# Bernat-C/MRI-Diffusion-SuperResolution

Hardware: AMD Instinct MI355X
Metric: MRI slices/sec (50-step DDIM, 256^2, bs=32) (higher is better)
Workload: dtype bf16; 1 GPU; configs[1]: 256x256 1-ch synthetic MRI slices -> 4x32x32 latents, SD-1.5-size UNet (859.5M params, random init) + rank-4 LoRA, 50-step DDIM, bs=32 per GPU; ddim_steps=50, parallelism=slice-sharded x1 (no collective), lora=explicit adapters, down-projection + rank-r update inside the projection GEMMs, tile_table=profiles/r03_tune_cache.tsv, hipgraph=True

## Files before the change

include/mrisr_debug.h:

```cpp
#ifndef MRISR_DEBUG_H
#define MRISR_DEBUG_H
#ifdef __cplusplus
extern "C" {
#endif

void mrisr_debug_force_split(int splitk);
void mrisr_debug_force_tile(int tile);
void mrisr_debug_prefer_tile(int tile);
void mrisr_debug_gemm_flags(int flags);
void mrisr_debug_set_tile_eff(int tile, double eff);
void mrisr_debug_set_tuned(const char* key, int tile, int splitk);
void mrisr_debug_gn_fused(int on);

int mrisr_autotune_stats(int* shapes, double* ms);
void mrisr_autotune_release(void);

int mrisr_bench_gemm(int M, int N, int K, int conv, int B, int H, int W, int stride, int ups, int c1, int tile, int splitk,
                     int iters, float* ms_out);

void mrisr_debug_sk_inkernel(int on);

void mrisr_debug_subpix(int min_rows);

void mrisr_debug_temb_table(int on);

void mrisr_debug_mlp_proj(int on);

void mrisr_debug_gn_slabs(int on);

void mrisr_debug_xattn_tail(int on);
void mrisr_debug_xattn_tail_stamps(void* dev_buf);

int mrisr_bench_mlp(int M, int hidden, int iters, float* ms_out);

#ifdef __cplusplus
}
#endif
#endif
```

mri-diffusion-superresolution_amd/csrc/common.h:

```cpp
#pragma once
#include <hip/hip_runtime.h>
#include <stdint.h>
#include <string>

namespace mrisr {

typedef __bf16 bf16;
typedef __attribute__((ext_vector_type(8))) __bf16 bf16x8;
typedef __attribute__((ext_vector_type(4))) __bf16 bf16x4;
typedef __attribute__((ext_vector_type(4))) float f32x4;
typedef __attribute__((ext_vector_type(16))) float f32x16;

enum DType : int { DT_F32 = 0, DT_BF16 = 1, DT_F16 = 2, DT_I64 = 3 };

template <typename T> struct TypeTag;
template <> struct TypeTag<float> { static constexpr int id = DT_F32; };
template <> struct TypeTag<bf16> { static constexpr int id = DT_BF16; };

__device__ __forceinline__ float to_f32(float x) { return x; }
__device__ __forceinline__ float to_f32(bf16 x) { return (float)x; }
template <typename T> __device__ __forceinline__ T from_f32(float x);
template <> __device__ __forceinline__ float from_f32<float>(float x) { return x; }
template <> __device__ __forceinline__ bf16 from_f32<bf16>(float x) { return (bf16)x; }

// ... 53 lines not shown
struct GemmArgs {
    const void* a0 = nullptr;
    const void* a1 = nullptr;
    int c0 = 0, c1 = 0;
    int lda0 = 0, lda1 = 0;
    int conv = 0;
    int B = 0, Hin = 0, Win = 0, Hout = 0, Wout = 0, stride = 1, ups = 0;
    int pad = 1;
    int zstuff = 0;
    const void* w = nullptr;
    int M = 0, N = 0, K = 0;
    int kw = 3, subpix = 0;
    int batch = 1;
    long long a_bs = 0, w_bs = 0;
    int heads = 1;
    long long o_bs = 0, o_hs = 0;
    int splitk = 1;
    float* partial = nullptr;
    unsigned* sk_counters = nullptr;
    int defer_reduce = 0;
    int pretouch = 0;
    float alpha = 1.0f;
    const float* bias = nullptr;
    const float* rowvec = nullptr;
    int rowvec_div = 1, rowvec_ld = 0;
    int act = ACT_NONE;
    const void* resid = nullptr;
    int ldr = 0;
    int out_mode = OUT_ROWS;
    void* out = nullptr;
    int ldo = 0;
    void* sec_ptr[3] = {nullptr, nullptr, nullptr};
    int sec_tr[3] = {0, 0, 0};
    int secC = 0, hd = 0, dpad = 0, ntok = 0, npad = 0, nheads = 0;
    double alg_flops = 0.0, alg_bytes = 0.0;
    int tile = 0;
    int stage_out = 1;
    const float* lora_z = nullptr;
    const float* lora_b = nullptr;
    int lora_r = 0, lora_zld = 0, lora_secN = 1;
    const void* lora_a = nullptr;
    int lora_R = 0;
    float* lora_zout = nullptr;
    const float* ln_gamma = nullptr;
    const float* ln_beta = nullptr;
    float ln_eps = 1e-5f;
    const void* w8 = nullptr;
    const float* w_scale = nullptr;
    const void* lora_a8 = nullptr;
    const float* lora_a_scale = nullptr;
    int no_rp = 0;
    int group_m = 1;
    int dbg = 0;
};

template <typename T> int launch_gemm(const GemmArgs& g, hipStream_t st);
template <typename T> int launch_splitk_reduce(const GemmArgs& g, hipStream_t st);
const void* zero_page();
int init_zero_page();
int gemm_prepare();
struct MlpArgs {
    const void* x = nullptr; int ldx = 0, M = 0;
    const float* ln_gamma = nullptr; const float* ln_beta = nullptr; float ln_eps = 1e-5f;
    const void* w1 = nullptr; const float* b1 = nullptr;
    const void* w2p = nullptr; const float* b2 = nullptr;
    const void* resid = nullptr; int ldr = 0;
    void* out = nullptr; int ldo = 0;
    int C = 0, H = 0, N2 = 0;
    const void* wp = nullptr; const float* bp = nullptr;
    const void* xres = nullptr; int ldxr = 0;
    void* out2 = nullptr; int ldo2 = 0;
};
bool mlp_fused_ok(int C, int H, int N2);
bool mlp_proj_enabled();
int launch_pack_mlp_w2(const void* w2_bf16, void* dst, int N2, int H, hipStream_t st);
int launch_mlp_fused(const MlpArgs& m, hipStream_t st);
struct XTailArgs {
    const void* ao = nullptr; int ldao = 0;
    void* t = nullptr; int ldt = 0;
    int M = 0, ntok = 0;
    const void* w1 = nullptr; const float* b1 = nullptr; const void* a1 = nullptr; const float* lb1 = nullptr;
    const float* ln_g = nullptr; const float* ln_b = nullptr; float ln_eps = 1e-5f;
    const void* wq = nullptr; const float* bq = nullptr; const void* aq = nullptr; const float* lbq = nullptr;
    const void* kvp = nullptr; int nk = 0; float scale = 1.f;
    const void* w2 = nullptr; const float* b2 = nullptr; const void* a2 = nullptr; const float* lb2 = nullptr;
    int lora_r = 0;
};
int xattn_tail_prepare();
bool xattn_tail_enabled();
bool xattn_tail_ok(int C, int heads, int M, int ntok, int nk);
size_t xattn_tail_kv_bytes(int B);
int launch_pack_xattn_kv(const void* kc, const void* vtc, void* dst, int B, int ctx_pad, int dpad, int nk, hipStream_t st);
int launch_xattn_tail(const XTailArgs& x, hipStream_t st);
int gemm_rp_tile(const GemmArgs& g);
int gemm_choose(GemmArgs& g, bool is_bf16);

struct GroupNormArgs {
    const void* x0 = nullptr;
    const void* x1 = nullptr;
    int c0 = 0, c1 = 0;
    int B = 0, HW = 0, groups = 32;
    float eps = 1e-5f;
    const float* gamma = nullptr;
    const float* beta = nullptr;
    int silu = 0;
    void* y = nullptr;
// ... 182 lines not shown
```

mri-diffusion-superresolution_amd/csrc/gemm.hip:

```cpp
#include "common.h"
#include "prof.h"

#include <cstdio>
#include <cstdlib>
#include <cstring>
#include <map>
#include <mutex>
#include <unordered_map>

namespace mrisr {

static void* g_zero_page = nullptr;
static constexpr size_t kZeroPageBytes = 128 * 1024;
const void* zero_page() { return g_zero_page; }
int init_zero_page() {
    if (g_zero_page) return 0;
    MRISR_CHECK_HIP(hipMalloc(&g_zero_page, kZeroPageBytes));
    MRISR_CHECK_HIP(hipMemset(g_zero_page, 0, kZeroPageBytes));
    return 0;
}

typedef const __attribute__((address_space(1))) void* gptr_t;
typedef __attribute__((address_space(3))) void* lptr_t;

// ... 115 lines not shown
    if (g.out_mode == OUT_NONE) {
        if (v[0] == 1.2345e30f) store4<T>(reinterpret_cast<T*>(g.out), v);
    } else if (g.out_mode == OUT_ROWS) {
        if (lds_dst) store4<T>(lds_dst, v);
        else store4<T>(reinterpret_cast<T*>(g.out) + zoff + (size_t)m * g.ldo + n0, v);
    } else if (g.out_mode == OUT_F32) {
        store4<float>(reinterpret_cast<float*>(g.out) + zoff + (size_t)m * g.ldo + n0, v);
    } else {
        if (lds_dst) {
            store4<T>(lds_dst, v);
            return;
        }
        if (sizeof(T) == 2 && lds_t) {
            unsigned w0, w1;
            const int drow = exchange_tokens4(v, w0, w1);
            *reinterpret_cast<uint2*>(lds_t + (nl + drow) * tpitch + (ml & ~3)) = make_uint2(w0, w1);
            return;
        }
        const int s = n0 / g.secC;
        const int c = n0 - s * g.secC;
        const int h = c / g.hd;
        const int dd = c - h * g.hd;
        const int b = m / g.ntok;
        const int tok = m - b * g.ntok;
        T* base = reinterpret_cast<T*>(s == 0 ? g.sec_ptr[0] : (s == 1 ? g.sec_ptr[1] : g.sec_ptr[2]));
        const int tr = (s == 0 ? g.sec_tr[0] : (s == 1 ? g.sec_tr[1] : g.sec_tr[2]));
        const size_t bh = (size_t)b * g.nheads + h;
        if (!tr) {
            store4<T>(base + (bh * g.npad + tok) * g.dpad + dd, v);
        } else if (sizeof(T) == 2 && mfma_lanes && (g.ntok & 3) == 0 && (g.M & 3) == 0) {
            unsigned w0, w1;
            const int drow = exchange_tokens4(v, w0, w1);
            T* o = base + (bh * g.dpad + dd + drow) * g.npad + (tok & ~3);
            *reinterpret_cast<uint2*>(o) = make_uint2(w0, w1);
        } else {
            T* o = base + (bh * g.dpad + dd) * g.npad + tok;
#pragma unroll
            for (int r = 0; r < 4; ++r) o[(size_t)r * g.npad] = from_f32<T>(v[r]);
        }
    }
}

template <int NFR>
__device__ __forceinline__ void preload_cols(const GemmArgs& g, int nbase, float (&pb)[NFR][4]) {
    const bool fold = g.rowvec && g.rowvec_div >= g.M;
#pragma unroll
    for (int i = 0; i < NFR; ++i) {
        const int n = min(nbase + i * 16, g.N - 4);
        float b[4] = {0.f, 0.f, 0.f, 0.f}, t[4] = {0.f, 0.f, 0.f, 0.f};
        if (g.bias) load4<float>(g.bias + n, b);
        if (fold) load4<float>(g.rowvec + n, t);
#pragma unroll
        for (int r = 0; r < 4; ++r) pb[i][r] = b[r] + t[r];
    }
}

template <typename T> struct Frag;
template <> struct Frag<bf16> { typedef bf16x8 type; };
template <> struct Frag<float> { typedef f32x4 type; };

__device__ __forceinline__ void mma(f32x4& acc, const bf16x8& w, const bf16x8& a) {
    acc = __builtin_amdgcn_mfma_f32_16x16x32_bf16(w, a, acc, 0, 0, 0);
}
__device__ __forceinline__ void mma(f32x4& acc, const f32x4& w, const f32x4& a) {
#pragma unroll
    for (int j = 0; j < 4; ++j) acc = __builtin_amdgcn_mfma_f32_16x16x4f32(w[j], a[j], acc, 0, 0, 0);
}

__device__ __forceinline__ void lds_poison(char* smem_base, int nthreads) {
    const unsigned bytes = ((const __attribute__((address_space(4))) unsigned*)__builtin_amdgcn_dispatch_ptr())[7];
    for (unsigned o = threadIdx.x * 16u; o + 16u <= bytes; o += (unsigned)nthreads * 16u)
        *reinterpret_cast<uint4*>(smem_base + o) = make_uint4(~0u, ~0u, ~0u, ~0u);
    __syncthreads();
}
static int gemm_flags_now();

template <typename T, int BM, int BN, int WGM, int WGN>
__global__ __launch_bounds__(256) void gemm_kernel(const GemmArgs g, const char* __restrict__ zero) {
    constexpr int EB = sizeof(T);
    constexpr int CH = 16 / EB;
    constexpr int BK = 8 * CH;
    constexpr int A_IT = BM / 32, W_IT = BN / 32;
    constexpr int WTM = BM / WGM, WTN = BN / WGN;
    constexpr int MF = WTM / 16, NF = WTN / 16;
    constexpr int STAGE = (BM + BN) * 128;
    static_assert(WGM * WGN == 4, "4 waves");
    extern __shared__ __attribute__((aligned(16))) char smem[];

    const int tid = threadIdx.x;
    const int lane = tid & 63;
    const int wave = __builtin_amdgcn_readfirstlane(tid >> 6);
    const int z = blockIdx.z;
    const int split = blockIdx.y;
    if (g.dbg & 2048) lds_poison(smem, (int)blockDim.x);

    const int ntn = (g.N + BN - 1) / BN;
    const int ntm = (g.M + BM - 1) / BM;
    const int nblk = ntn * ntm;
    int logical;
    {
        const int bid = blockIdx.x;
        const int xcd = bid & 7, q = nblk >> 3, r = nblk & 7;
        logical = (xcd < r ? xcd * (q + 1) : r * (q + 1) + (xcd - r) * q) + (bid >> 3);
    }
    int tn, tm;
    {
// ... 237 lines not shown
template <int BM, int BN>
__device__ __forceinline__ void copy_out_heads(const GemmArgs& g, const bf16* otile, int m0, int n0, bool tr) {
    __syncthreads();
    const int s = n0 / g.secC;
    bf16* base = reinterpret_cast<bf16*>(s == 0 ? g.sec_ptr[0] : (s == 1 ? g.sec_ptr[1] : g.sec_ptr[2]));
    if (!tr) {
        constexpr int CPR = BN / 8, P = BN + 8;
        for (int idx = threadIdx.x; idx < BM * CPR; idx += 256) {
            const int row = idx / CPR, ch = idx - row * CPR;
            const int m = m0 + row, n = n0 + ch * 8;
            if (m >= g.M || n >= g.N) continue;
            const int c = n - s * g.secC, h = c / g.hd, dd = c - h * g.hd;
            const int b = m / g.ntok, tok = m - b * g.ntok;
            *reinterpret_cast<bf16x8*>(base + (((size_t)b * g.nheads + h) * g.npad + tok) * g.dpad + dd) =
                *reinterpret_cast<const bf16x8*>(otile + row * P + ch * 8);
        }
    } else {
        constexpr int TPC = BM / 8, P = BM + 8;
        for (int idx = threadIdx.x; idx < BN * TPC; idx += 256) {
            const int col = idx / TPC, tc = idx - col * TPC;
            const int n = n0 + col, m = m0 + tc * 8;
            if (m >= g.M || n >= g.N) continue;
            const int c = n - s * g.secC, h = c / g.hd, dd = c - h * g.hd;
            const int b = m / g.ntok, tok = m - b * g.ntok;
            *reinterpret_cast<bf16x8*>(base + (((size_t)b * g.nheads + h) * g.dpad + dd) * g.npad + tok) =
                *reinterpret_cast<const bf16x8*>(otile + col * P + tc * 8);
        }
    }
}

typedef __attribute__((address_space(3))) void* lds_ptr_t;
__device__ __forceinline__ __amdgpu_buffer_rsrc_t make_rsrc(const void* p, unsigned bytes) {
    return __builtin_amdgcn_make_buffer_rsrc(const_cast<void*>(p), 0, bytes, 0x00020000);
}
__device__ __forceinline__ void bl16(__amdgpu_buffer_rsrc_t r, char* lds_wave_base, unsigned voff, unsigned soff) {
    __builtin_amdgcn_raw_ptr_buffer_load_lds(r, (lds_ptr_t)lds_wave_base, 16, voff, soff, 0, 0);
}
#define BL_OOB 0x80000000u


__device__ __forceinline__ void pretouch_weights(const __amdgpu_buffer_rsrc_t& rw, long long w_bytes, char* scratch, int wave, int lane, int cap) {
    const int n_wg = (int)(gridDim.x * gridDim.y);
    const int wg = (int)(blockIdx.x + blockIdx.y * gridDim.x);
    const long long pieces = (w_bytes + 1023) >> 10;
    const int per_wg = (int)((pieces + n_wg - 1) / n_wg);
    const int per_wave = min((per_wg + 3) >> 2, cap);
    const long long first = (long long)wg * per_wg + (long long)wave * per_wave;
    for (int i = 0; i < per_wave; ++i) {
        const long long pc = first + i;
        const unsigned off = pc < pieces ? (unsigned)(pc << 10) + (unsigned)lane * 16u : BL_OOB;
        bl16(rw, scratch + ((wave * 2 + (i & 1)) << 10), off, 0u);
    }
}

template <int NF, int MF>
__device__ __forceinline__ bool splitk_last_arriver(const GemmArgs& g, f32x4 (&acc)[NF][MF], unsigned tile_idx, const float* slab0, int m_base, int n_base,
                                                    int fr, int fg, char* ticket_lds) {
    __builtin_amdgcn_fence(__ATOMIC_RELEASE, "agent");
    __syncthreads();
    if (threadIdx.x == 0)
        *reinterpret_cast<volatile unsigned*>(ticket_lds) = __hip_atomic_fetch_add(g.sk_counters + tile_idx, 1u, __ATOMIC_ACQ_REL, __HIP_MEMORY_SCOPE_AGENT);
    __syncthreads();
    const unsigned ticket = *reinterpret_cast<volatile unsigned*>(ticket_lds);
    if (ticket != (unsigned)g.splitk - 1) return false;
    __syncthreads();
    if (threadIdx.x == 0) __hip_atomic_store(g.sk_counters + tile_idx, 0u, __ATOMIC_RELAXED, __HIP_MEMORY_SCOPE_AGENT);
    __builtin_amdgcn_fence(__ATOMIC_ACQUIRE, "agent");
    const size_t slab = (size_t)g.M * g.N;
#pragma unroll
    for (int i = 0; i < NF; ++i)
#pragma unroll
        for (int j = 0; j < MF; ++j) acc[i][j] = f32x4{0.f, 0.f, 0.f, 0.f};
    for (int s = 0; s < g.splitk; ++s) {
        const float* p = slab0 + (size_t)s * slab;
#pragma unroll
        for (int i = 0; i < NF; ++i)
#pragma unroll
            for (int j = 0; j < MF; ++j) {
                const int m = m_base + j * 16 + fr;
                const int n = n_base + i * 16 + fg * 4;
                if (m < g.M && n < g.N) {
                    const f32x4 t = __builtin_nontemporal_load(reinterpret_cast<const f32x4*>(p + (size_t)m * g.N + n));
                    acc[i][j] += t;
                }
            }
    }
    return true;
}

template <int BM, int BN, int WGM, int WGN, int NSTAGE, bool LORA>
__global__ __launch_bounds__(256, 2) void gemm_bl_kernel(const GemmArgs g) {
    static_assert(NSTAGE >= 2 && NSTAGE <= 4, "2 (drain per tile), 3 or 4 (counted ring)");
    typedef bf16 T;
    constexpr int BK = 64;
    constexpr int A_IT = BM / 32, W_IT = BN / 32;
    constexpr int WTM = BM / WGM, WTN = BN / WGN;
    constexpr int MF = WTM / 16, NF = WTN / 16;
    constexpr int STAGE = (BM + BN) * 128 + (LORA ? 16 * 128 : 0);
    static_assert(WGM * WGN == 4, "4 waves");
    extern __shared__ __attribute__((aligned(16))) char smem[];

    const int tid = threadIdx.x;
    const int lane = tid & 63;
    const int wave = __builtin_amdgcn_readfirstlane(tid >> 6);
    const int z = blockIdx.z;
    const int split = blockIdx.y;
    if (g.dbg & 2048) lds_poison(smem, (int)blockDim.x);

    const int ntn = (g.N + BN - 1) / BN;
    const int ntm = (g.M + BM - 1) / BM;
    const int nblk = ntn * ntm;
    int logical;
    {
        const int bid = blockIdx.x;
        const int xcd = bid & 7, q = nblk >> 3, r = nblk & 7;
        logical = (xcd < r ? xcd * (q + 1) : r * (q + 1) + (xcd - r) * q) + (bid >> 3);
    }
    int tn, tm;
    {
        const int GM = g.group_m > 1 ? g.group_m : 1;
        const int per_group = GM * ntn;
        const int grp = logical / per_group;
        const int first_m = grp * GM;
        const int gsz = min(GM, ntm - first_m);
        const int within = logical - grp * per_group;
        tm = first_m + within % gsz;
        tn = within / gsz;
    }
    const int m0 = tm * BM, n0 = tn * BN;

    const T* a0p = reinterpret_cast<const T*>(g.a0) + (size_t)z * g.a_bs;
    const T* a1p = reinterpret_cast<const T*>(g.a1);
    const T* wp = reinterpret_cast<const T*>(g.w) + (size_t)z * g.w_bs;
    const long long a_rows = g.conv ? (long long)g.B * g.Hin * g.Win : (long long)g.M;
    const __amdgpu_buffer_rsrc_t rw = make_rsrc(wp, (unsigned)min((long long)g.N * g.K * 2, 0x7FFFFFFFll));
    const __amdgpu_buffer_rsrc_t ra0 = make_rsrc(a0p, (unsigned)min(a_rows * g.lda0 * 2, 0x7FFFFFFFll));
    const __amdgpu_buffer_rsrc_t ra1 = make_rsrc(a1p ? (const void*)a1p : (const void*)a0p,
                                                 a1p ? (unsigned)min(a_rows * g.lda1 * 2, 0x7FFFFFFFll) : 0u);

    const int lrow = tid >> 3, pch = tid & 7;
    unsigned wvo[W_IT];
#pragma unroll
    for (int it = 0; it < W_IT; ++it) {
        const int row = it * 32 + lrow;
        const int n = n0 + row;
        const int c = pch ^ (row & 7);
        wvo[it] = n < g.N ? (unsigned)(((size_t)n * g.K + c * 8) * 2) : BL_OOB;
    }
    unsigned avo[A_IT], avo1[A_IT];
    int ab[A_IT], ay[A_IT], ax[A_IT];
#pragma unroll
    for (int it = 0; it < A_IT; ++it) {
        const int row = it * 32 + lrow;
        const int m = m0 + row;
        const int c = pch ^ (row & 7);
        const bool ok = m < g.M;
        avo[it] = avo1[it] = BL_OOB;
        ab[it] = -1;
        ay[it] = ax[it] = 0;
// ... 66 lines not shown
                for (int it = 0; it < A_IT; ++it) {
                    const int row = it * 32 + lrow;
                    const int c = pch ^ (row & 7);
                    const int iy = ay[it] + ky, ix = ax[it] + kx;
                    const bool ok = ab[it] >= 0 && iy >= 0 && iy < Hc && ix >= 0 && ix < Wc && (!g.zstuff || ((iy | ix) & 1) == 0);
                    const unsigned pix = (unsigned)((ab[it] + (iy >> g.ups)) * g.Win + (ix >> g.ups));
                    avo[it] = ok ? (pix * (unsigned)ld + (unsigned)c * 8u) * 2u : BL_OOB;
                }
            }
            const unsigned chb = (unsigned)(second ? cc - g.c0 : cc) * 2;
            if (!second) {
#pragma unroll
                for (int it = 0; it < A_IT; ++it) bl16(ra0, sb + (it * 256 + wave * 64) * 16, avo[it], chb);
            } else {
#pragma unroll
                for (int it = 0; it < A_IT; ++it) bl16(ra1, sb + (it * 256 + wave * 64) * 16, avo[it], chb);
            }
            cc += BK;
            if (cc >= Ct) { cc = 0; ++tap; }
        }
    };
    auto stage = [&](int kt, int buf) { stage_w(kt, buf); stage_a(kt, buf); };
    (void)acb;

    f32x4 acc[NF][MF];
#pragma unroll
    for (int i = 0; i < NF; ++i)
#pragma unroll
        for (int j = 0; j < MF; ++j) acc[i][j] = f32x4{0.f, 0.f, 0.f, 0.f};

    const int wm0 = (wave / WGN) * WTM, wn0 = (wave % WGN) * WTN;
    const int fr = lane & 15, fg = lane >> 4;
    const bool zwave = LORA && (wave % WGN) == 0;
    const bool lora_mma = LORA && g.lora_r == 4 && g.alpha == 1.0f && !(g.dbg & 8);
    bf16x8 lbf[NF];
    if (LORA) {
#pragma unroll
        for (int i = 0; i < NF; ++i) {
            lbf[i] = bf16x8{0, 0, 0, 0, 0, 0, 0, 0};
            const int n = n0 + wn0 + i * 16 + fr;
            if (lora_mma && n < g.N) {
                const int sec = n / g.lora_secN;
                if ((sec >> 1) == fg) {
                    const f32x4 l = *reinterpret_cast<const f32x4*>(g.lora_b + (size_t)n * 4);
                    if (sec & 1) { lbf[i][4] = (bf16)l[0]; lbf[i][5] = (bf16)l[1]; lbf[i][6] = (bf16)l[2]; lbf[i][7] = (bf16)l[3]; }
                    else { lbf[i][0] = (bf16)l[0]; lbf[i][1] = (bf16)l[1]; lbf[i][2] = (bf16)l[2]; lbf[i][3] = (bf16)l[3]; }
                }
            }
        }
    }
    f32x4 zacc[MF];
#pragma unroll
    for (int j = 0; j < MF; ++j) zacc[j] = f32x4{0.f, 0.f, 0.f, 0.f};

    auto compute = [&](int buf, auto&& mid) {
        const char* sa = smem + buf * STAGE;
        const char* sw = sa + BM * 128;
#pragma unroll
        for (int kk = 0; kk < 2; ++kk) {
            if (kk == 1) mid();
            const int phys = ((kk * 4 + fg) ^ (fr & 7)) * 16;
            bf16x8 wf[NF], af[MF];
#pragma unroll
            for (int i = 0; i < NF; ++i) wf[i] = *reinterpret_cast<const bf16x8*>(sw + (wn0 + i * 16 + fr) * 128 + phys);
#pragma unroll
            for (int j = 0; j < MF; ++j) af[j] = *reinterpret_cast<const bf16x8*>(sa + (wm0 + j * 16 + fr) * 128 + phys);
#pragma unroll
            for (int i = 0; i < NF; ++i)
#pragma unroll
                for (int j = 0; j < MF; ++j) acc[i][j] = __builtin_amdgcn_mfma_f32_16x16x32_bf16(wf[i], af[j], acc[i][j], 0, 0, 0);
            if (LORA && zwave) {
                const bf16x8 lf = *reinterpret_cast<const bf16x8*>(sw + (BN + fr) * 128 + phys);
#pragma unroll
                for (int j = 0; j < MF; ++j) zacc[j] = __builtin_amdgcn_mfma_f32_16x16x32_bf16(lf, af[j], zacc[j], 0, 0, 0);
            }
        }
    };

    if constexpr (NSTAGE == 2) {
        if (kt_beg < kt_end) {
            if (g.pretouch) pretouch_weights(rw, (long long)g.N * g.K * 2, smem + STAGE, wave, lane, g.pretouch);
            stage(kt_beg, 0);
            asm volatile("s_waitcnt vmcnt(0)" ::: "memory");
            __syncthreads();
            int cur = 0;
            const bool halves = (g.dbg & 16384) != 0;
            for (int kt = kt_beg; kt < kt_end; ++kt) {
                const bool more = kt + 1 < kt_end;
                if (more) { if (halves) stage_w(kt + 1, cur ^ 1); else stage(kt + 1, cur ^ 1); }
                compute(cur, [&]() {
                    if (halves) {
                        __builtin_amdgcn_sched_barrier(0);
                        if (more) stage_a(kt + 1, cur ^ 1);
                        __builtin_amdgcn_sched_barrier(0);
                    }
                });
                asm volatile("s_waitcnt vmcnt(0)" ::: "memory");
                __syncthreads();
                cur ^= 1;
            }
        }
    } else {
        constexpr int PER = A_IT + W_IT + (LORA ? 1 : 0);
        static_assert(PER * (NSTAGE - 2) <= 63, "vmcnt range");
#pragma unroll
        for (int s = 0; s < NSTAGE - 1; ++s)
            if (kt_beg + s < kt_end) stage(kt_beg + s, s);
        int slot = 0;
        for (int kt = kt_beg; kt < kt_end; ++kt) {
            const int younger = min(NSTAGE - 2, kt_end - 1 - kt);
            if (younger >= 2) asm volatile("s_waitcnt vmcnt(%0)" ::"n"(PER * 2) : "memory");
            else if (younger == 1) asm volatile("s_waitcnt vmcnt(%0)" ::"n"(PER) : "memory");
            else asm volatile("s_waitcnt vmcnt(0)" ::: "memory");
            asm volatile("s_waitcnt lgkmcnt(0)" ::: "memory");
            __builtin_amdgcn_s_barrier();
            if (kt + NSTAGE - 1 < kt_end) stage(kt + NSTAGE - 1, (slot + NSTAGE - 1) % NSTAGE);
            compute(slot, []() {});
            slot = slot + 1 == NSTAGE ? 0 : slot + 1;
        }
        __syncthreads();
    }

    float* zlds = reinterpret_cast<float*>(smem);
    if (LORA) {
        if (zwave) {
#pragma unroll
            for (int j = 0; j < MF; ++j) {
                const int ml = wm0 + j * 16 + fr;
                *reinterpret_cast<f32x4*>(zlds + ml * 16 + fg * 4) = zacc[j];
                if (g.lora_zout && tn == 0 && m0 + ml < g.M && fg * 4 < g.lora_R)
                    *reinterpret_cast<f32x4*>(g.lora_zout + (size_t)(m0 + ml) * g.lora_R + fg * 4) = zacc[j];
            }
        }
        __syncthreads();
    }
    if (LORA && lora_mma) {
        bf16x8 zf[MF];
#pragma unroll
        for (int j = 0; j < MF; ++j) {
            zf[j] = bf16x8{0, 0, 0, 0, 0, 0, 0, 0};
            if (fg < 2) {
                const float* zp = zlds + (wm0 + j * 16 + fr) * 16 + fg * 8;
                const f32x4 a = *reinterpret_cast<const f32x4*>(zp), b = *reinterpret_cast<const f32x4*>(zp + 4);
                zf[j] = bf16x8{(bf16)a[0], (bf16)a[1], (bf16)a[2], (bf16)a[3], (bf16)b[0], (bf16)b[1], (bf16)b[2], (bf16)b[3]};
            }
        }
#pragma unroll
        for (int i = 0; i < NF; ++i)
#pragma unroll
            for (int j = 0; j < MF; ++j) acc[i][j] = __builtin_amdgcn_mfma_f32_16x16x32_bf16(lbf[i], zf[j], acc[i][j], 0, 0, 0);
    }
    if (g.splitk > 1) {
        float* part = g.partial + ((size_t)z * g.splitk + split) * (size_t)g.M * g.N;
#pragma unroll
        for (int i = 0; i < NF; ++i)
#pragma unroll
            for (int j = 0; j < MF; ++j) {
                const int m = m0 + wm0 + j * 16 + fr;
                const int n = n0 + wn0 + i * 16 + fg * 4;
                if (m < g.M && n < g.N) {
                    float v[4] = {acc[i][j][0], acc[i][j][1], acc[i][j][2], acc[i][j][3]};
                    store4<float>(part + (size_t)m * g.N + n, v);
                }
            }
        if constexpr (NF * MF > 20) return;
        else {
            if (!g.sk_counters) return;
            if (!splitk_last_arriver<NF, MF>(g, acc, (unsigned)(z * gridDim.x + blockIdx.x), g.partial + (size_t)z * g.splitk * (size_t)g.M * g.N,
                                             m0 + wm0, n0 + wn0, fr, fg, smem))
                return;
        }
    }
    float pb[NF][4];
    preload_cols<NF>(g, n0 + wn0 + fg * 4, pb);
    if (g.act == ACT_GEGLU) {
        if constexpr (NF % 2 == 0) {
#pragma unroll
            for (int i = 0; i < NF; i += 2)
#pragma unroll
                for (int j = 0; j < MF; ++j) {
                    const int m = m0 + wm0 + j * 16 + fr;
                    const int n = n0 + wn0 + i * 16 + fg * 4;
                    if (m < g.M && n < g.N) {
                        float v[4] = {acc[i][j][0], acc[i][j][1], acc[i][j][2], acc[i][j][3]};
                        float vg[4] = {acc[i + 1][j][0], acc[i + 1][j][1], acc[i + 1][j][2], acc[i + 1][j][3]};
                        epilogue4<T>(g, z, m, n, v, vg, nullptr, nullptr, false, true, nullptr, 0, 0, 0, pb[i], pb[i + 1]);
                    }
                }
        }
        return;
    }
    constexpr int OPITCH = BN + 8;
    T* otile = reinterpret_cast<T*>(smem + (LORA ? BM * 16 * 4 : 0));
    const bool staged = g.out_mode == OUT_ROWS && (g.ldo & 7) == 0 && g.heads == 1 && g.stage_out;
    const bool resid_later = staged && g.resid != nullptr && (g.ldr & 7) == 0 && g.stage_out < 3;
    bool hstaged = false, htr = false;
    if (g.out_mode == OUT_HEADS && g.stage_out && !(g.dbg & 16)) {
        const int sec = n0 / g.secC;
        hstaged = (min(n0 + BN, g.N) - 1) / g.secC == sec && ((g.N | g.M | g.hd | g.secC | g.dpad | g.npad | g.ntok) & 7) == 0 && g.heads == 1 &&
                  g.batch == 1;
        htr = (sec == 0 ? g.sec_tr[0] : (sec == 1 ? g.sec_tr[1] : g.sec_tr[2])) != 0;
    }
#pragma unroll
    for (int i = 0; i < NF; ++i)
#pragma unroll
        for (int j = 0; j < MF; ++j) {
            const int m = m0 + wm0 + j * 16 + fr;
            const int n = n0 + wn0 + i * 16 + fg * 4;
            if (m < g.M && n < g.N) {
                float v[4] = {acc[i][j][0], acc[i][j][1], acc[i][j][2], acc[i][j][3]};
                epilogue4<T>(g, z, m, n, v, nullptr, LORA && !lora_mma ? zlds + (m - m0) * 16 : nullptr,
                             staged || (hstaged && !htr) ? otile + (m - m0) * OPITCH + (n - n0) : nullptr, resid_later, true,
                             hstaged && htr ? otile : nullptr, m - m0, n - n0, BM + 8, pb[i]);
            }
        }
    if (staged) copy_out_tile<BM, BN>(g, otile, OPITCH, m0, n0, z, resid_later);
    else if (hstaged) copy_out_heads<BM, BN>(g, otile, m0, n0, htr);
}

template <int BM, int BN, int WGM, int WGN>
__global__ __launch_bounds__(256, 2) void gemm_halo_kernel(const GemmArgs g) {
    typedef bf16 T;
    constexpr int BK = 64;
    constexpr int W_IT = BN / 32;
    constexpr int WTM = BM / WGM, WTN = BN / WGN;
    constexpr int MF = WTM / 16, NF = WTN / 16;
    constexpr int WSTAGE = BN * 128;
    constexpr int PIT_MAX = (BM >= 256 ? 13 : (BM >= 128 ? 9 : 6));
    static_assert(WGM * WGN == 4, "4 waves");
    extern __shared__ __attribute__((aligned(16))) char smem[];

    const int tid = threadIdx.x;
    const int lane = tid & 63;
    const int wave = __builtin_amdgcn_readfirstlane(tid >> 6);
    const int split = blockIdx.y;
    if (g.dbg & 2048) lds_poison(smem, (int)blockDim.x);
    const int Wd = g.Win, Hd = g.Hin;
    const int TH = BM / Wd, PW = Wd + 2;
    const int npix = (TH + 2) * PW;
    const int pit = (npix * 8 + 255) / 256;
    char* patch = smem;
    char* wbase = smem + pit * 4096;

    const int ntn = (g.N + BN - 1) / BN;
    const int ntm = g.M / BM;
    const int nblk = ntn * ntm;
    int logical;
    {
        const int bid = blockIdx.x;
        const int xcd = bid & 7, q = nblk >> 3, r = nblk & 7;
        logical = (xcd < r ? xcd * (q + 1) : r * (q + 1) + (xcd - r) * q) + (bid >> 3);
    }
    int tn, tm;
    {
        const int GM = g.group_m > 1 ? g.group_m : 1;
        const int per_group = GM * ntn;
        const int grp = logical / per_group;
        const int first_m = grp * GM;
        const int gsz = min(GM, ntm - first_m);
        const int within = logical - grp * per_group;
        tm = first_m + within % gsz;
        tn = within / gsz;
    }
    const int m0 = tm * BM, n0 = tn * BN;
    const int img = m0 / (Hd * Wd);
    const int y0 = (m0 - img * Hd * Wd) / Wd;

    const T* a0p = reinterpret_cast<const T*>(g.a0);
    const T* a1p = reinterpret_cast<const T*>(g.a1);
    const T* wp = reinterpret_cast<const T*>(g.w);
// ... 1453 lines not shown
}

static int auto_group_m(int ntm, int ntn, int BM, int BN) {
    (void)ntn; (void)BM; (void)BN;
    static const int env = [] { const char* e = getenv("MRISR_GROUP_M"); return e ? atoi(e) : 8; }();
    return std::max(1, std::min(env, ntm));
}

template <typename T, int BM, int BN, int WGM, int WGN>
static int prepare_cfg() {
    constexpr int smem = 2 * (BM + BN) * 128;
    static bool attr_set = false;
    if (!attr_set) {
        auto kern = gemm_kernel<T, BM, BN, WGM, WGN>;
        MRISR_CHECK_HIP(hipFuncSetAttribute((const void*)kern, hipFuncAttributeMaxDynamicSharedMemorySize, smem));
        attr_set = true;
    }
    return 0;
}
template <typename T>
static int prepare_all() {
    if (prepare_cfg<T, 128, 128, 2, 2>()) return 1;
    if (prepare_cfg<T, 256, 64, 4, 1>()) return 1;
    if (prepare_cfg<T, 128, 64, 2, 2>()) return 1;
    if (prepare_cfg<T, 64, 64, 2, 2>()) return 1;
    return 0;
}
template <typename T, int BM, int BN, int WGM, int WGN>
static int launch_cfg(const GemmArgs& g, hipStream_t st) {
    constexpr int smem = 2 * (BM + BN) * 128;
    auto kern = gemm_kernel<T, BM, BN, WGM, WGN>;
    if (prepare_cfg<T, BM, BN, WGM, WGN>()) return 1;
    const int ntn = (g.N + BN - 1) / BN, ntm = (g.M + BM - 1) / BM;
    const_cast<GemmArgs&>(g).group_m = auto_group_m(ntm, ntn, BM, BN);
    dim3 grid(ntn * ntm, g.splitk, g.batch);
    static const std::string pname = std::string("gemm_") + (sizeof(T) == 2 ? "bf16_" : "f32_") + std::to_string(BM) + "x" + std::to_string(BN);
    double fl = g.alg_flops, by = g.alg_bytes;
    if (prof_enabled()) {
        if (fl == 0.0) fl = 2.0 * g.M * (double)g.N * g.K * g.batch;
        if (by == 0.0) {
            const double a_el = g.conv ? (double)g.B * g.Hin * g.Win * (g.c0 + g.c1) : (double)g.M * g.K;
            by = sizeof(T) * g.batch * (a_el + (double)g.N * g.K + (double)g.M * g.N);
        }
    }
    ProfScope ps(pname.c_str(), fl, by, st);
    hipLaunchKernelGGL(kern, grid, dim3(256), smem, st, g, (const char*)zero_page());
    MRISR_CHECK_HIP(hipGetLastError());
    return 0;
}

static int g_force_tile = 0;
extern "C" void mrisr_debug_force_tile(int t) { g_force_tile = t; }

template <int BM, int BN, int WGM, int WGN, int NSTAGE>
static int prepare_bl() {
    constexpr int smem = NSTAGE * (BM + BN) * 128;
    constexpr int smem_l = NSTAGE * ((BM + BN) * 128 + 16 * 128);
    static bool done = false;
    if (!done) {
        MRISR_CHECK_HIP(hipFuncSetAttribute((const void*)gemm_bl_kernel<BM, BN, WGM, WGN, NSTAGE, false>, hipFuncAttributeMaxDynamicSharedMemorySize, smem));
        MRISR_CHECK_HIP(hipFuncSetAttribute((const void*)gemm_bl_kernel<BM, BN, WGM, WGN, NSTAGE, true>, hipFuncAttributeMaxDynamicSharedMemorySize, smem_l));
        done = true;
    }
    return 0;
}
template <int BM, int BN, int WGM, int WGN, int NSTAGE>
static int launch_bl(const GemmArgs& g, hipStream_t st) {
    constexpr int smem = NSTAGE * (BM + BN) * 128;
    constexpr int smem_l = NSTAGE * ((BM + BN) * 128 + 16 * 128);
    if (prepare_bl<BM, BN, WGM, WGN, NSTAGE>()) return 1;
    if (NSTAGE > 2)
        MRISR_REQUIRE(!g.conv && !g.c1 && !g.a1 && g.batch == 1 && (g.splitk == 1 || (g.K / 64) / g.splitk >= NSTAGE) && g.M % BM == 0 && g.N % BN == 0,
                      "counted-ring GEMM: plain single-source GEMM that tiles exactly; split: at least NSTAGE K tiles per split");
    const int ntn = (g.N + BN - 1) / BN, ntm = (g.M + BM - 1) / BM;
    const_cast<GemmArgs&>(g).group_m = auto_group_m(ntm, ntn, BM, BN);
    dim3 grid(ntn * ntm, g.splitk, g.batch);
    static const std::string base_name = std::string("gemm_bf16_bl") + std::to_string(BM) + "x" + std::to_string(BN) + (NSTAGE > 2 ? "d" + std::to_string(NSTAGE) : std::string());
    std::string pname = base_name;
    if (prof_enabled() && prof_shapes()) {
        char buf[160];
        snprintf(buf, sizeof(buf), "%s %s M=%d N=%d K=%d s=%d b=%d", base_name.c_str(), g.conv ? (g.ups ? "convup" : (g.stride == 2 ? "convs2" : "conv")) : "lin",
                 g.M, g.N, g.K, g.splitk, g.batch);
        pname = buf;
    }
    double fl = g.alg_flops, by = g.alg_bytes;
    if (prof_enabled()) {
        if (fl == 0.0) fl = 2.0 * g.M * (double)g.N * g.K * g.batch;
        if (by == 0.0) {
            const double a_el = g.conv ? (double)g.B * g.Hin * g.Win * (g.c0 + g.c1) : (double)g.M * g.K;
            by = 2.0 * g.batch * (a_el + (double)g.N * g.K + (double)g.M * g.N);
        }
    }
    ProfScope ps(prof_intern(pname), fl, by, st);
    if (g.lora_a) {
        MRISR_REQUIRE(g.splitk == 1 && !g.conv && g.c1 == 0 && g.lora_R >= 1 && g.lora_R <= 16 && g.lora_b && g.act != ACT_GEGLU,
                      "in-kernel LoRA down-projection: plain un-split GEMM, R <= 16");
        hipLaunchKernelGGL((gemm_bl_kernel<BM, BN, WGM, WGN, NSTAGE, true>), grid, dim3(256), smem_l, st, g);
    } else {
        hipLaunchKernelGGL((gemm_bl_kernel<BM, BN, WGM, WGN, NSTAGE, false>), grid, dim3(256), smem, st, g);
    }
    MRISR_CHECK_HIP(hipGetLastError());
    return 0;
}
#define BL_CFGS(X)             \
    X(14, 128, 128, 2, 2, 2)   \
    X(15, 256, 64, 4, 1, 2)    \
    X(16, 128, 64, 2, 2, 2)    \
    X(17, 64, 64, 2, 2, 2)     \
    X(18, 64, 128, 2, 2, 2)    \
    X(25, 128, 160, 2, 2, 2)   \
    X(26, 64, 160, 2, 2, 2)    \
    X(27, 160, 160, 2, 2, 2)   \
    X(28, 128, 192, 2, 2, 2)   \
    X(29, 192, 128, 2, 2, 2)   \
    X(30, 160, 128, 2, 2, 2)   \
    X(31, 96, 160, 2, 2, 2)    \
    X(32, 64, 64, 2, 2, 4)     \
    X(33, 64, 64, 2, 2, 3)     \
    X(34, 64, 128, 2, 2, 3)    \
    X(35, 128, 64, 2, 2, 3)    \
    X(36, 128, 128, 2, 2, 3)   \
    X(37, 128, 160, 2, 2, 4)   \
    X(38, 128, 128, 2, 2, 4)   \
    X(39, 64, 160, 2, 2, 3)

static int prepare_bls() {
#define X(id, bm, bn, wm, wn, ns) if (prepare_bl<bm, bn, wm, wn, ns>()) return 1;
    BL_CFGS(X)
#undef X
    return 0;
}
#define HALO_CFGS(X)        \
    X(41, 128, 160, 2, 2)   \
    X(42, 128, 128, 2, 2)   \
    X(43, 64, 160, 2, 2)    \
    X(44, 128, 192, 2, 2)   \
    X(45, 256, 64, 4, 1)

static size_t halo_smem(const GemmArgs& g, int BM, int BN) {
    const int TH = BM / g.Win;
    const size_t npix = (size_t)(TH + 2) * (g.Win + 2);
    const size_t patch = (npix * 8 + 255) / 256 * 4096;
    return patch + 2 * (size_t)BN * 128;
}
static bool halo_ok(const GemmArgs& g, int BM) {
    if (!g.conv || g.stride != 1 || g.ups != 0 || g.zstuff || g.batch != 1 || g.pad != 1) return false;
// ... 616 lines not shown
```

mri-diffusion-superresolution_amd/mrisr/_lib.py:

```python
from __future__ import annotations

import ctypes as C
import os
from typing import Optional, Sequence

import torch

_HERE = os.path.dirname(os.path.abspath(__file__))
LIB_PATH = os.path.join(os.path.dirname(_HERE), "csrc", "libmrisr.so")

MRISR_F32, MRISR_BF16, MRISR_F16, MRISR_I64 = 0, 1, 2, 3
MRISR_NCHW, MRISR_NHWC = 0, 1
STEP_DDIM, STEP_RESSHIFT, STEP_DDPM, STEP_UNIPC, STEP_DPMSOLVERPP = 0, 1, 2, 3, 4
ACT_NONE, ACT_RELU, ACT_SILU, ACT_GEGLU = 0, 1, 2, 3

_DT = {torch.float32: MRISR_F32, torch.bfloat16: MRISR_BF16, torch.float16: MRISR_F16, torch.int64: MRISR_I64}


class Tensor(C.Structure):
    _fields_ = [("data", C.c_void_p), ("dtype", C.c_int32), ("layout", C.c_int32), ("ndim", C.c_int32),
                ("shape", C.c_int64 * 4)]


class UNetCfg(C.Structure):
    _fields_ = [("in_channels", C.c_int32), ("out_channels", C.c_int32), ("num_levels", C.c_int32),
                ("block_out_channels", C.c_int32 * 4), ("attn_levels", C.c_int32 * 4),
                ("layers_per_block", C.c_int32), ("num_heads", C.c_int32), ("cross_attention_dim", C.c_int32),
                ("norm_num_groups", C.c_int32), ("norm_eps", C.c_float), ("cond_channels", C.c_int32),
                ("cond_embed_channels", C.c_int32 * 4), ("compute_dtype", C.c_int32), ("lora_rank", C.c_int32),
                ("lora_fused", C.c_int32), ("flash_attention", C.c_int32), ("fp8_linears", C.c_int32),
                ("fp8_attention", C.c_int32), ("fp8_train", C.c_int32)]


class AdapterCfg(C.Structure):
    _fields_ = [("channels", C.c_int32 * 4), ("nums_rb", C.c_int32), ("cin", C.c_int32), ("ksize", C.c_int32),
                ("use_conv", C.c_int32), ("compute_dtype", C.c_int32)]


class VaeCfg(C.Structure):
    _fields_ = [("in_channels", C.c_int32), ("out_channels", C.c_int32), ("latent_channels", C.c_int32),
                ("num_levels", C.c_int32), ("block_out_channels", C.c_int32 * 4), ("layers_per_block", C.c_int32),
                ("norm_num_groups", C.c_int32), ("compute_dtype", C.c_int32), ("scaling_factor", C.c_float)]


class MrisrError(RuntimeError):
    pass


_lib: Optional[C.CDLL] = None

EXPORTS = [
    "mrisr_last_error", "mrisr_version", "mrisr_unet_create", "mrisr_controlnet_create", "mrisr_model_destroy",
    "mrisr_model_set_param", "mrisr_model_set_lora_scale", "mrisr_model_finalize", "mrisr_model_num_params",
    "mrisr_model_workspace_bytes", "mrisr_unet_forward", "mrisr_model_set_context", "mrisr_model_num_skips",
    "mrisr_model_skip_shape", "mrisr_controlnet_forward", "mrisr_controlnet_set_cond", "mrisr_adapter_create",
    "mrisr_adapter_destroy", "mrisr_adapter_set_param", "mrisr_adapter_finalize", "mrisr_adapter_forward",
    "mrisr_resshift_forward", "mrisr_sampler_create", "mrisr_sampler_destroy", "mrisr_sampler_run", "mrisr_sampler_set_range", "mrisr_sampler_set_clip",
    "mrisr_sampler_set_guidance", "mrisr_sampler_run_guided", "mrisr_op_guided_step", "mrisr_sampler_set_solver", "mrisr_op_multistep_step",
    "mrisr_adapter_train_prepare", "mrisr_adapter_train_num_trainable", "mrisr_adapter_train_num_tensors",
    "mrisr_adapter_train_tensor_info", "mrisr_adapter_train_bind", "mrisr_adapter_train_refresh", "mrisr_adapter_backward", "mrisr_adapter_backward_level", "mrisr_adapter_train_level_range",
    "mrisr_vae_create", "mrisr_vae_destroy", "mrisr_vae_set_param", "mrisr_vae_num_params", "mrisr_vae_finalize",
    "mrisr_vae_encode", "mrisr_vae_decode",
# ... 118 lines not shown
```

Measured before the change: 66.10 slices/s.

## Overlap weight pretouch with first stage and issue bias loads before main loop

In the two-stage bl GEMM, the kernel now stages the first K tile before the L2 pretouch of weights. The pretouch writes into its own 1 KB LDS scratch, and the kernel waits only until the stage loads are done (a partial vmcnt wait) instead of draining every load, so the pretouch traffic no longer delays the first compute. Bias and rowvec column loads for the epilogue are issued before the main loop, hiding their latency behind it. The cost is extra LDS per block, which can reduce occupancy, and more registers held live through the loop. The change also adds optional cycle-stamp instrumentation, compiled out by default, and an environment override for the library path.

After: 64.58 slices/s. -2.3%, worse.

```diff
diff --git a/include/mrisr_debug.h b/include/mrisr_debug.h
--- a/include/mrisr_debug.h
+++ b/include/mrisr_debug.h
@@ -8,6 +8,7 @@
 void mrisr_debug_force_tile(int tile);
 void mrisr_debug_prefer_tile(int tile);
 void mrisr_debug_gemm_flags(int flags);
+void mrisr_debug_bl_stamps(void* dev_buf, int slots, int wg_cap, int M, int N, int K, int lora);
 void mrisr_debug_set_tile_eff(int tile, double eff);
 void mrisr_debug_set_tuned(const char* key, int tile, int splitk);
 void mrisr_debug_gn_fused(int on);
diff --git a/mri-diffusion-superresolution_amd/csrc/common.h b/mri-diffusion-superresolution_amd/csrc/common.h
--- a/mri-diffusion-superresolution_amd/csrc/common.h
+++ b/mri-diffusion-superresolution_amd/csrc/common.h
@@ -129,6 +129,7 @@
     int no_rp = 0;
     int group_m = 1;
     int dbg = 0;
+    unsigned long long* stamps = nullptr;
 };
 
 template <typename T> int launch_gemm(const GemmArgs& g, hipStream_t st);
diff --git a/mri-diffusion-superresolution_amd/csrc/gemm.hip b/mri-diffusion-superresolution_amd/csrc/gemm.hip
--- a/mri-diffusion-superresolution_amd/csrc/gemm.hip
+++ b/mri-diffusion-superresolution_amd/csrc/gemm.hip
@@ -191,6 +191,19 @@
         if (fold) load4<float>(g.rowvec + n, t);
 #pragma unroll
         for (int r = 0; r < 4; ++r) pb[i][r] = b[r] + t[r];
+    }
+}
+
+template <int NFR>
+__device__ __forceinline__ void preload_cols_issue(const GemmArgs& g, int nbase, float (&b)[NFR][4], float (&t)[NFR][4]) {
+    const bool fold = g.rowvec && g.rowvec_div >= g.M;
+#pragma unroll
+    for (int i = 0; i < NFR; ++i) {
+        const int n = min(nbase + i * 16, g.N - 4);
+#pragma unroll
+        for (int r = 0; r < 4; ++r) b[i][r] = t[i][r] = 0.f;
+        if (g.bias) load4<float>(g.bias + n, b[i]);
+        if (fold) load4<float>(g.rowvec + n, t[i]);
     }
 }
 
@@ -534,6 +547,24 @@
         bl16(rw, scratch + ((wave * 2 + (i & 1)) << 10), off, 0u);
     }
 }
+__device__ __forceinline__ int pretouch_weights_in_range(const __amdgpu_buffer_rsrc_t& rw, long long w_bytes, char* scratch, int wave, int lane, int cap) {
+    const int n_wg = (int)(gridDim.x * gridDim.y);
+    const int wg = (int)(blockIdx.x + blockIdx.y * gridDim.x);
+    const long long pieces = (w_bytes + 1023) >> 10;
+    const int per_wg = (int)((pieces + n_wg - 1) / n_wg);
+    const int per_wave = min((per_wg + 3) >> 2, cap);
+    const long long first = (long long)wg * per_wg + (long long)wave * per_wave;
+    const int n = (int)max(0ll, min((long long)per_wave, pieces - first));
+    for (int i = 0; i < n; ++i) bl16(rw, scratch, (unsigned)((first + i) << 10) + (unsigned)lane * 16u, 0u);
+    return n;
+}
+__device__ __forceinline__ void wait_vmcnt_at_most(int n) {
+#define MRISR_VMCNT_CASE(k) if (n >= k) { asm volatile("s_waitcnt vmcnt(" #k ")" ::: "memory"); return; }
+    MRISR_VMCNT_CASE(32) MRISR_VMCNT_CASE(24) MRISR_VMCNT_CASE(16) MRISR_VMCNT_CASE(12) MRISR_VMCNT_CASE(8) MRISR_VMCNT_CASE(6)
+    MRISR_VMCNT_CASE(5) MRISR_VMCNT_CASE(4) MRISR_VMCNT_CASE(3) MRISR_VMCNT_CASE(2) MRISR_VMCNT_CASE(1)
+#undef MRISR_VMCNT_CASE
+    asm volatile("s_waitcnt vmcnt(0)" ::: "memory");
+}
 
 template <int NF, int MF>
 __device__ __forceinline__ bool splitk_last_arriver(const GemmArgs& g, f32x4 (&acc)[NF][MF], unsigned tile_idx, const float* slab0, int m_base, int n_base,
@@ -570,6 +601,12 @@
     return true;
 }
 
+constexpr int BL_PT_BYTES = 1024;
+__host__ __device__ constexpr bool bl_pretouch_own(int BM, int BN, int NSTAGE) {
+    return NSTAGE == 2 && 2 * (2 * ((BM + BN) * 128 + 16 * 128) + BL_PT_BYTES) <= 160 * 1024;
+}
+constexpr int BL_NSTAMP = 16;
+
 template <int BM, int BN, int WGM, int WGN, int NSTAGE, bool LORA>
 __global__ __launch_bounds__(256, 2) void gemm_bl_kernel(const GemmArgs g) {
     static_assert(NSTAGE >= 2 && NSTAGE <= 4, "2 (drain per tile), 3 or 4 (counted ring)");
@@ -579,6 +616,7 @@
     constexpr int WTM = BM / WGM, WTN = BN / WGN;
     constexpr int MF = WTM / 16, NF = WTN / 16;
     constexpr int STAGE = (BM + BN) * 128 + (LORA ? 16 * 128 : 0);
+    constexpr bool PT_OWN = bl_pretouch_own(BM, BN, NSTAGE);
     static_assert(WGM * WGN == 4, "4 waves");
     extern __shared__ __attribute__((aligned(16))) char smem[];
 
@@ -587,6 +625,33 @@
     const int wave = __builtin_amdgcn_readfirstlane(tid >> 6);
     const int z = blockIdx.z;
     const int split = blockIdx.y;
+#ifdef MRISR_BL_STAMPS
+    unsigned long long st_[BL_NSTAMP];
+    const bool st_on = g.stamps != nullptr && wave == 0;
+#pragma unroll
+    for (int k = 0; k < BL_NSTAMP; ++k) st_[k] = 0;
+    unsigned long long st_w0_ = 0;
+#define BL_STAMP(k) do { if (st_on) st_[k] = __builtin_readcyclecounter(); } while (0)
+#define BL_WAIT_BEGIN() do { if (st_on) st_w0_ = __builtin_readcyclecounter(); } while (0)
+#define BL_WAIT_END() do { if (st_on) { st_[12] += __builtin_readcyclecounter() - st_w0_; st_[13] += 1; } } while (0)
+#define BL_STAMP_FLUSH()                                                                                                           \
+    do {                                                                                                                          \
+        if (st_on) {                                                                                                              \
+            asm volatile("s_waitcnt vmcnt(0)" ::: "memory");                                                                      \
+            st_[11] = __builtin_readcyclecounter();                                                                               \
+            if (lane == 0) {                                                                                                      \
+                unsigned long long* o_ = g.stamps + ((size_t)(blockIdx.z * gridDim.y + blockIdx.y) * gridDim.x + blockIdx.x) * BL_NSTAMP; \
+                for (int k = 0; k < BL_NSTAMP; ++k) o_[k] = st_[k];                                                                \
+            }                                                                                                                     \
+        }                                                                                                                         \
+    } while (0)
+    BL_STAMP(0);
+#else
+#define BL_STAMP(k) do {} while (0)
+#define BL_WAIT_BEGIN() do {} while (0)
+#define BL_WAIT_END() do {} while (0)
+#define BL_STAMP_FLUSH() do {} while (0)
+#endif
     if (g.dbg & 2048) lds_poison(smem, (int)blockDim.x);
 
     const int ntn = (g.N + BN - 1) / BN;
@@ -759,6 +824,9 @@
     f32x4 zacc[MF];
 #pragma unroll
     for (int j = 0; j < MF; ++j) zacc[j] = f32x4{0.f, 0.f, 0.f, 0.f};
+    const bool cols_early = g.splitk == 1 && !(g.dbg & 65536);
+    float pb_b[NF][4], pb_t[NF][4];
+    if (cols_early) preload_cols_issue<NF>(g, n0 + wn0 + fg * 4, pb_b, pb_t);
 
     auto compute = [&](int buf, auto&& mid) {
         const char* sa = smem + buf * STAGE;
@@ -786,10 +854,37 @@
 
     if constexpr (NSTAGE == 2) {
         if (kt_beg < kt_end) {
-            if (g.pretouch) pretouch_weights(rw, (long long)g.N * g.K * 2, smem + STAGE, wave, lane, g.pretouch);
-            stage(kt_beg, 0);
-            asm volatile("s_waitcnt vmcnt(0)" ::: "memory");
-            __syncthreads();
+            BL_STAMP(1);
+            if (PT_OWN && g.pretouch && !(g.dbg & 32768)) {
+                stage(kt_beg, 0);
+                bool in_range = true;
+                {
+                    const bool second = !g.conv && kt_beg * BK >= g.c0;
+#pragma unroll
+                    for (int it = 0; it < W_IT; ++it) in_range = in_range && __builtin_amdgcn_ballot_w64(wvo[it] != BL_OOB) != 0;
+#pragma unroll
+                    for (int it = 0; it < A_IT; ++it) in_range = in_range && __builtin_amdgcn_ballot_w64((second ? avo1[it] : avo[it]) != BL_OOB) != 0;
+                    if (LORA && wave < 2) in_range = in_range && __builtin_amdgcn_ballot_w64(lvo != BL_OOB) != 0;
+                }
+                char* pt = smem + NSTAGE * STAGE;
+                if (in_range) {
+                    const int n = pretouch_weights_in_range(rw, (long long)g.N * g.K * 2, pt, wave, lane, g.pretouch);
+                    BL_STAMP(2);
+                    wait_vmcnt_at_most(n);
+                } else {
+                    BL_STAMP(2);
+                    asm volatile("s_waitcnt vmcnt(0)" ::: "memory");
+                    (void)pretouch_weights_in_range(rw, (long long)g.N * g.K * 2, pt, wave, lane, g.pretouch);
+                }
+                __builtin_amdgcn_s_barrier();
+            } else {
+                if (g.pretouch) pretouch_weights(rw, (long long)g.N * g.K * 2, smem + STAGE, wave, lane, g.pretouch);
+                stage(kt_beg, 0);
+                BL_STAMP(2);
+                asm volatile("s_waitcnt vmcnt(0)" ::: "memory");
+                __syncthreads();
+            }
+            BL_STAMP(3);
             int cur = 0;
             const bool halves = (g.dbg & 16384) != 0;
             for (int kt = kt_beg; kt < kt_end; ++kt) {
@@ -802,10 +897,13 @@
                         __builtin_amdgcn_sched_barrier(0);
                     }
                 });
+                BL_WAIT_BEGIN();
                 asm volatile("s_waitcnt vmcnt(0)" ::: "memory");
                 __syncthreads();
+                BL_WAIT_END();
                 cur ^= 1;
             }
+            BL_STAMP(4);
         }
     } else {
         constexpr int PER = A_IT + W_IT + (LORA ? 1 : 0);
@@ -828,6 +926,7 @@
         __syncthreads();
     }
 
+    BL_STAMP(5);
     float* zlds = reinterpret_cast<float*>(smem);
     if (LORA) {
         if (zwave) {
@@ -857,6 +956,7 @@
 #pragma unroll
             for (int j = 0; j < MF; ++j) acc[i][j] = __builtin_amdgcn_mfma_f32_16x16x32_bf16(lbf[i], zf[j], acc[i][j], 0, 0, 0);
     }
+    BL_STAMP(6);
     if (g.splitk > 1) {
         float* part = g.partial + ((size_t)z * g.splitk + split) * (size_t)g.M * g.N;
 #pragma unroll
@@ -870,16 +970,28 @@
                     store4<float>(part + (size_t)m * g.N + n, v);
                 }
             }
-        if constexpr (NF * MF > 20) return;
+        BL_STAMP(9);
+        if constexpr (NF * MF > 20) { BL_STAMP_FLUSH(); return; }
         else {
-            if (!g.sk_counters) return;
+            if (!g.sk_counters) { BL_STAMP_FLUSH(); return; }
             if (!splitk_last_arriver<NF, MF>(g, acc, (unsigned)(z * gridDim.x + blockIdx.x), g.partial + (size_t)z * g.splitk * (size_t)g.M * g.N,
                                              m0 + wm0, n0 + wn0, fr, fg, smem))
                 return;
         }
     }
     float pb[NF][4];
-    preload_cols<NF>(g, n0 + wn0 + fg * 4, pb);
+    if (cols_early) {
+#pragma unroll
+        for (int i = 0; i < NF; ++i)
+#pragma unroll
+            for (int r = 0; r < 4; ++r) pb[i][r] = pb_b[i][r] + pb_t[i][r];
+    } else {
+        preload_cols<NF>(g, n0 + wn0 + fg * 4, pb);
+    }
+#ifdef MRISR_BL_STAMPS
+    if (st_on) asm volatile("s_waitcnt vmcnt(0)" ::: "memory");
+#endif
+    BL_STAMP(7);
     if (g.act == ACT_GEGLU) {
         if constexpr (NF % 2 == 0) {
 #pragma unroll
@@ -895,6 +1007,8 @@
                     }
                 }
         }
+        BL_STAMP(9);
+        BL_STAMP_FLUSH();
         return;
     }
     constexpr int OPITCH = BN + 8;
@@ -921,8 +1035,15 @@
                              hstaged && htr ? otile : nullptr, m - m0, n - n0, BM + 8, pb[i]);
             }
         }
+    BL_STAMP(8);
     if (staged) copy_out_tile<BM, BN>(g, otile, OPITCH, m0, n0, z, resid_later);
     else if (hstaged) copy_out_heads<BM, BN>(g, otile, m0, n0, htr);
+    BL_STAMP(9);
+    BL_STAMP_FLUSH();
+#undef BL_STAMP
+#undef BL_WAIT_BEGIN
+#undef BL_WAIT_END
+#undef BL_STAMP_FLUSH
 }
 
 template <int BM, int BN, int WGM, int WGN>
@@ -2482,10 +2603,22 @@
 static int g_force_tile = 0;
 extern "C" void mrisr_debug_force_tile(int t) { g_force_tile = t; }
 
+struct BlStampSel { unsigned long long* buf; int slots, wg_cap, M, N, K, lora, next; };
+static BlStampSel g_bl_stamps = {nullptr, 0, 0, 0, 0, 0, -1, 0};
+extern "C" void mrisr_debug_bl_stamps(void* dev_buf, int slots, int wg_cap, int M, int N, int K, int lora) {
+    g_bl_stamps = BlStampSel{static_cast<unsigned long long*>(dev_buf), slots, wg_cap, M, N, K, lora, 0};
+}
+static unsigned long long* bl_stamp_slot(const GemmArgs& g, long long wgs) {
+    auto& s = g_bl_stamps;
+    if (!s.buf || s.next >= s.slots || wgs > s.wg_cap || g.M != s.M || g.N != s.N || g.K != s.K || (s.lora >= 0 && s.lora != (g.lora_a ? 1 : 0))) return nullptr;
+    return s.buf + (size_t)(s.next++) * s.wg_cap * BL_NSTAMP;
+}
+
 template <int BM, int BN, int WGM, int WGN, int NSTAGE>
 static int prepare_bl() {
-    constexpr int smem = NSTAGE * (BM + BN) * 128;
-    constexpr int smem_l = NSTAGE * ((BM + BN) * 128 + 16 * 128);
+    constexpr int pt = bl_pretouch_own(BM, BN, NSTAGE) ? BL_PT_BYTES : 0;
+    constexpr int smem = NSTAGE * (BM + BN) * 128 + pt;
+    constexpr int smem_l = NSTAGE * ((BM + BN) * 128 + 16 * 128) + pt;
     static bool done = false;
     if (!done) {
         MRISR_CHECK_HIP(hipFuncSetAttribute((const void*)gemm_bl_kernel<BM, BN, WGM, WGN, NSTAGE, false>, hipFuncAttributeMaxDynamicSharedMemorySize, smem));
@@ -2496,8 +2629,9 @@
 }
 template <int BM, int BN, int WGM, int WGN, int NSTAGE>
 static int launch_bl(const GemmArgs& g, hipStream_t st) {
-    constexpr int smem = NSTAGE * (BM + BN) * 128;
-    constexpr int smem_l = NSTAGE * ((BM + BN) * 128 + 16 * 128);
+    constexpr int pt = bl_pretouch_own(BM, BN, NSTAGE) ? BL_PT_BYTES : 0;
+    constexpr int smem = NSTAGE * (BM + BN) * 128 + pt;
+    constexpr int smem_l = NSTAGE * ((BM + BN) * 128 + 16 * 128) + pt;
     if (prepare_bl<BM, BN, WGM, WGN, NSTAGE>()) return 1;
     if (NSTAGE > 2)
         MRISR_REQUIRE(!g.conv && !g.c1 && !g.a1 && g.batch == 1 && (g.splitk == 1 || (g.K / 64) / g.splitk >= NSTAGE) && g.M % BM == 0 && g.N % BN == 0,
@@ -2522,6 +2656,7 @@
         }
     }
     ProfScope ps(prof_intern(pname), fl, by, st);
+    const_cast<GemmArgs&>(g).stamps = bl_stamp_slot(g, (long long)grid.x * grid.y * grid.z);
     if (g.lora_a) {
         MRISR_REQUIRE(g.splitk == 1 && !g.conv && g.c1 == 0 && g.lora_R >= 1 && g.lora_R <= 16 && g.lora_b && g.act != ACT_GEGLU,
                       "in-kernel LoRA down-projection: plain un-split GEMM, R <= 16");
diff --git a/mri-diffusion-superresolution_amd/mrisr/_lib.py b/mri-diffusion-superresolution_amd/mrisr/_lib.py
--- a/mri-diffusion-superresolution_amd/mrisr/_lib.py
+++ b/mri-diffusion-superresolution_amd/mrisr/_lib.py
@@ -7,7 +7,7 @@
 import torch
 
 _HERE = os.path.dirname(os.path.abspath(__file__))
-LIB_PATH = os.path.join(os.path.dirname(_HERE), "csrc", "libmrisr.so")
+LIB_PATH = os.environ.get("MRISR_LIB") or os.path.join(os.path.dirname(_HERE), "csrc", "libmrisr.so")
 
 MRISR_F32, MRISR_BF16, MRISR_F16, MRISR_I64 = 0, 1, 2, 3
 MRISR_NCHW, MRISR_NHWC = 0, 1
```
